# kubernetes-sigs/karpenter

Hardware: AMD Instinct MI355X
Metric: pods scheduled/sec (Solve()) (higher is better)
Workload: dtype int64

## Files before the change

### karpenter_amd/csrc/fast_engine.h

```cpp
#pragma once
#include <type_traits>
#include "kernels.h"
#include "pdq_emul.h"

namespace ks {

constexpr int kFastRows = 4;
constexpr uint32_t kFastFree = 0xFFFFFFFFu;
constexpr uint32_t kFastLastBit = 0x80000000u;
constexpr int kFastEnt = 1024;
constexpr int kFastPool = 256;
constexpr int kFastMaxPareto = 16;
constexpr int kFastMaxVar = 12;
constexpr uint64_t kFastExtBit = 1ull << 63;
constexpr int kFastVarBits = 56;

struct FastClaim { uint64_t vmask; int32_t req[4]; };
template <int R> struct FastRec { uint64_t vmask; int32_t req[4]; uint64_t acc[R]; };
struct FastSlot { uint64_t cvmask; uint64_t dmask; int32_t size[4]; uint32_t tmplok; uint32_t kdef; };
struct FastEnt { uint64_t vmask; int32_t cap[4]; uint32_t info; uint32_t pad; };

struct FastPlan {
  int total_bytes, cap;
  int off_state, off_key, off_ord, off_snap, off_ent, off_pool, off_slot, off_misc, off_hot;
// ... 40 lines not shown
  uint16_t* o_snap;
  uint64_t* c_rec;
  uint32_t* cls_first;
  uint32_t* cls_last;
  uint32_t* max_active;
  FastNodes* nodes;
  uint32_t* nd_pod;
  const uint64_t* nd_dead0;
  FastPlan plan;
  int enabled;
};

typedef uint64_t __attribute__((may_alias)) u64_alias;
template <class T>
KS_FN T lds_get(const KS_LDS T* p) {
  static_assert(sizeof(T) % 8 == 0, "lds_get: 8-byte multiples");
  T out;
  u64_alias* o = (u64_alias*)&out;
  const KS_LDS u64_alias* s = (const KS_LDS u64_alias*)p;
#pragma unroll
  for (int i = 0; i < (int)(sizeof(T) / 8); ++i) o[i] = s[i];
  return out;
}
template <class T>
KS_FN void lds_put(KS_LDS T* p, const T& v) {
  static_assert(sizeof(T) % 8 == 0, "lds_put: 8-byte multiples");
  const u64_alias* o = (const u64_alias*)&v;
  KS_LDS u64_alias* s = (KS_LDS u64_alias*)p;
#pragma unroll
  for (int i = 0; i < (int)(sizeof(T) / 8); ++i) s[i] = o[i];
}


typedef uint32_t __attribute__((vector_size(16), may_alias)) u32x4_alias;
template <class T>
KS_FN T lds_get16(const KS_LDS T* p) {
  static_assert(sizeof(T) % 16 == 0, "lds_get16: 16-byte multiples");
  T out;
  u32x4_alias* o = (u32x4_alias*)&out;
  const KS_LDS u32x4_alias* s = (const KS_LDS u32x4_alias*)p;
#pragma unroll
  for (int i = 0; i < (int)(sizeof(T) / 16); ++i) o[i] = s[i];
  return out;
}
KS_FN FastEnt ent_live(const KS_LDS FastEnt* p) {
  FastEnt out;
  *(u32x4_alias*)&out = *(const KS_LDS u32x4_alias*)p;
  *(u64_alias*)&out.cap[2] = *(const KS_LDS u64_alias*)&p->cap[2];
  out.info = 1; out.pad = 0;
  return out;
}
template <class T>
KS_FN void lds_put16(KS_LDS T* p, const T& v) {
  static_assert(sizeof(T) % 16 == 0, "lds_put16: 16-byte multiples");
  const u32x4_alias* o = (const u32x4_alias*)&v;
  KS_LDS u32x4_alias* s = (KS_LDS u32x4_alias*)p;
#pragma unroll
  for (int i = 0; i < (int)(sizeof(T) / 16); ++i) s[i] = o[i];
}

template <bool HBM, int R> struct ClaimRecs;
template <int R> struct ClaimRecs<false, R> {
  KS_LDS FastRec<R>* p;
  KS_FN FastClaim state(uint32_t c) const { return lds_get((const KS_LDS FastClaim*)&p[c]); }
  KS_FN void put_state(uint32_t c, const FastClaim& v) const { lds_put((KS_LDS FastClaim*)&p[c], v); }
  KS_FN uint64_t acc(uint32_t c, int row) const { return p[c].acc[row]; }
  KS_FN void put_acc(uint32_t c, int row, uint64_t v) const { p[c].acc[row] = v; }
// ... 167 lines not shown
  uint32_t helper;
  uint32_t simd[4];
};
#if KS_DEVICE
KS_FN uint32_t mail_load(const KS_LDS uint32_t* p) { return *(const volatile KS_LDS uint32_t*)p; }
KS_FN void mail_store(KS_LDS uint32_t* p, uint32_t v) { *(volatile KS_LDS uint32_t*)p = v; }
#else
KS_FN uint32_t mail_load(const uint32_t* p) { return *p; }
KS_FN void mail_store(uint32_t* p, uint32_t v) { *p = v; }
#endif

struct FastHot {
  alignas(16) FastMail mail;
  int base, bi, bn, n, np, max_steps, steps, status;
  int pend_a, pend_x, pend_new, ev_arg;
  uint32_t pend_mv;
  int rf_x;
  int rf_x2;
  unsigned long long n_steps, n_tests, n_ref, hot_cycles;
  unsigned long long tsec[8];
  unsigned long long hw[4];
  const uint32_t* q_class; const volatile int* cancel; uint32_t* q_claim; uint32_t* q_cnt;
  uint32_t cur[kFastRows][64];
  uint32_t scls[kFastRows][64];
  uint32_t bcls[64], oclaim[64], ocnt[64], nxt_cls[64];
};

template <class W, int GS, int R>
struct FastCold {
  const ProblemView* Pk;
  const Workspace* Sk;
  const FastWork* Fk;
  typedef typename FastMem<GS, R>::o16 o16;
  ClaimOrder<W, o16, false> order;
  typename FastMem<GS, R>::s16 snap;
  typename FastMem<GS, R>::States cst;
  KS_LDS FastEnt* ent;
  KS_LDS int32_t* pool;
  KS_LDS FastSlot* aslot;
  KS_LDS FastMisc* Mp;
  KS_LDS FastHot* hs;
  int n_claims = 0, nv = 0, n_ent = 0, n_pool = 0, n_evict = 0;
  uint32_t host_seq = 0, active_templates = 0;
  int bail_code = 0;
  int lo_ = 0, hi_ = -1;
  unsigned long long n_ref_extra = 0, n_cold_tests = 0;

  KS_DEV void init(const ProblemView* p, const Workspace* s, const FastWork* f, char* lds) {
    Pk = p; Sk = s; Fk = f;
    const FastPlan& pl = f->plan;
    Mp = (KS_LDS FastMisc*)(lds + pl.off_misc);
    hs = (KS_LDS FastHot*)(lds + pl.off_hot);
    if constexpr (GS >= 1) cst.p = (FastRec<R>*)f->c_rec; else cst.p = (KS_LDS FastRec<R>*)(lds + pl.off_state);
    typedef typename FastMem<GS, R>::s16 s16;
    if constexpr (GS >= 2) { order.key = (o16)f->o_key; order.ord = (o16)f->o_ord; }
    else { order.key = (o16)(lds + pl.off_key); order.ord = (o16)(lds + pl.off_ord); }
    if constexpr (GS >= 1) snap = (s16)f->o_snap; else snap = (s16)(lds + pl.off_snap);
    order.pos = nullptr;
    ent = (KS_LDS FastEnt*)(lds + pl.off_ent);
    pool = (KS_LDS int32_t*)(lds + pl.off_pool);
    aslot = (KS_LDS FastSlot*)(lds + pl.off_slot);
  }

  KS_COLD int create_entry(uint64_t vm) {
    vm = W::uniform(vm);
    const ProblemView& P = *Pk; const Workspace& S = *Sk; const FastWork& F = *Fk;
    const int t = (int)(vm >> 56);
    const int iw = P.it_words, n_its = P.n_its, nr = P.n_res;
    const Dict& d = P.dict;
    const ProblemView& Pv = P;
    KS_LDS FastMisc& Mm = *Mp;
    const uint64_t* tits = S.t_its + (size_t)t * iw;
    KS_LDS uint64_t* its = Mp->its;
    const int nvv = nv;
    W::for_n(iw, [&](int w) {
      uint64_t acc = tits[w];
      for (int j = 0; j < nvv; ++j) {
        const int k = Mm.vkey[j];
        if (!((Pv.it_keys >> k) & 1u)) continue;
// ... 309 lines not shown
      while (todo) {
        LaneVar<uint64_t> missv;
        const uint64_t td = todo;
        uint64_t okb = 0, miss = 0, d0, d1;
        W::ballot4([&](int l) {
          missv.at(l) = 0;
          if (!((td >> l) & 1)) return 0;
          const FastClaim st = cs_.state((uint32_t)(x0 + l));
          if (!((rec.tmplok >> (st.vmask >> 56)) & 1u)) return 0;
          const uint64_t m = st.vmask & rec.cvmask;
          if (!fast_fields_ok(m, rec.dmask)) return 0;
          FastEnt e;
          if (fast_lookup(ent, m, e) < 0) { missv.at(l) = m; return 2; }
          return fast_fits(pool, e, st.req, rec.size) ? 1 : 0;
        }, okb, miss, d0, d1);
        accm |= okb;
        todo = miss;
        if (miss && create_entry(missv.bcast(ctz64(miss))) < 0) { bail_code = DECLINE_CACHE_FULL; return -1; }
      }
      W::each([&](int l) {
        if (x0 + l < nc) {
          const uint64_t w = cs_.acc((uint32_t)(x0 + l), row);
          cs_.put_acc((uint32_t)(x0 + l), row, (w & ~bit) | (((accm >> l) & 1) ? bit : 0ull));
        }
      });
    }
    W::sync();
    return slot | evicted;
  }

  KS_COLD void slow_sort(int n, int defect, int app) {
    order.n = (int)W::uniform((uint64_t)(uint32_t)n); order.defect = (int)W::uniform((uint64_t)(uint32_t)defect); order.defect_append = W::uniform((uint64_t)app) != 0;
    n = order.n;
    const o16 oo = order.ord; const typename FastMem<GS, R>::s16 sn = snap;
    if constexpr (FastMem<GS, R>::kSnapHbm) {
      W::copy8(sn, oo, n);
      order.sort();
      lo_ = W::find_first8(0, n, [&](int i) { return sn[i] != oo[i]; });
      if (lo_ >= n) { lo_ = 0; hi_ = -1; return; }
      hi_ = W::find_last8(0, n, [&](int i) { return sn[i] != oo[i]; });
    } else {
      const int n8 = (n + 7) >> 3;
      const KS_LDS u32x4_alias* const o8 = (const KS_LDS u32x4_alias*)oo;
      KS_LDS u32x4_alias* const s8 = (KS_LDS u32x4_alias*)sn;
      W::for_n(n8, [&](int i) { s8[i] = o8[i]; });
      order.sort();
      auto differs = [&](int i) { const u32x4_alias a = s8[i], b = o8[i]; return ((a[0] ^ b[0]) | (a[1] ^ b[1]) | (a[2] ^ b[2]) | (a[3] ^ b[3])) != 0; };
      const int c0 = W::find_first(0, n8, differs);
      if (c0 >= n8) { lo_ = 0; hi_ = -1; return; }
      const int c1 = W::find_last(0, n8, differs);
      lo_ = W::find_first(c0 * 8, c0 * 8 + 8 < n ? c0 * 8 + 8 : n, [&](int i) { return sn[i] != oo[i]; });
      hi_ = W::find_last(c1 * 8, c1 * 8 + 8 < n ? c1 * 8 + 8 : n, [&](int i) { return sn[i] != oo[i]; });
    }
  }
  KS_DEV void shift_right16(KS_LDS uint16_t* arr, int b, int a) {
    KS_LDS u32x4_alias* const v = (KS_LDS u32x4_alias*)arr;
    const KS_LDS uint32_t* const dw = (const KS_LDS uint32_t*)arr;
    for (int e0 = a & ~511; e0 >= 0 && e0 + 511 >= b; e0 -= 512) {
      LaneVar<uint32_t> d0, d1, d2, d3, pv;
      const uint32_t below = e0 > 0 ? dw[(e0 >> 1) - 1] : 0u;
      W::each([&](int l) {
        const int e = e0 + 8 * l;
        d0.at(l) = 0; d1.at(l) = 0; d2.at(l) = 0; d3.at(l) = 0;
        if (e <= a && e + 7 >= b) { const u32x4_alias x = v[(e0 >> 3) + l]; d0.at(l) = x[0]; d1.at(l) = x[1]; d2.at(l) = x[2]; d3.at(l) = x[3]; }
      });
      LaneVar<uint32_t> up;
      W::each([&](int l) { up.at(l) = d3.shuffle(l, (l + 63) & 63); });
// ... 80 lines not shown
    }
    bail_code = DECLINE_UNSCHEDULABLE_POD;
    return 0;
  }

  KS_COLD void finish(int status, int n, unsigned long long steps, unsigned long long n_steps, unsigned long long n_tests, unsigned long long n_ref, const unsigned long long* tc) {
    const Workspace& S = *Sk; const FastWork& F = *Fk;
    if (status != 3 && status != 1) {
      uint32_t* go = S.o_ord;
      const o16 oo = order.ord; const o16 ok_ = order.key;
      FastClaim* gs = F.c_state; uint32_t* gn = F.c_npods; uint16_t* ge = F.c_ent;
      const typename FastMem<GS, R>::States ls = cst;
      const KS_LDS FastEnt* en = ent;
      W::for_n(n, [&](int i) { const uint32_t c = oo[i]; go[i] = c; gn[c] = ok_[i]; });
      W::for_n(n, [&](int c) {
        const FastClaim st = ls.state((uint32_t)c);
        FastEnt e;
        gs[c] = st;
        ge[c] = (uint16_t)fast_lookup(en, st.vmask, e);
      });
      W::store(S.n_claims_out, n_claims);
    }
    FastNodes nd{};
    if (F.nodes) nd = *F.nodes;
    if (status == 0 && nd.limit_hit) status = 2;
    if (status) W::store(S.status_out, status);
    Counters c{};
    c.bin_evaluations = n_tests + n_cold_tests + nd.n_tests; c.full_evaluations = n_steps; c.queue_pops = steps + nd.n_placed; c.sorts = steps; c.slow_sorts = order.slow_sorts;
    c.column_resets = (unsigned long long)n_evict; c.ref_bin_evaluations = n_ref + n_ref_extra + nd.n_ref;
    c.decline = (unsigned long long)(bail_code > 0 ? bail_code : 0);
    if (tc) for (int i = 0; i < 16; ++i) c.cycles[i] = tc[i];
#ifdef KSOLVE_PHASE_TIMERS
    for (int i = 0; i < 4; ++i) c.cycles[16 + i] = hs->hw[i];
    c.cycles[18] = (hs->hw[2] << 32) | (unsigned long long)(hs->mail.simd[0] | (hs->mail.simd[1] << 8) | (hs->mail.simd[2] << 16) | (hs->mail.simd[3] << 24));
#endif
    if (F.nodes) c.cycles[19] = (unsigned long long)nd.variant;
    if (W::leader()) *S.counters = c;
    W::sync();
  }
};

template <int GS, int R>
struct FastHotCtx {
  typename FastMem<GS, R>::o16 okey, oord; typename FastMem<GS, R>::States cst; KS_LDS FastEnt* ent; KS_LDS int32_t* pool;
  KS_LDS FastSlot* aslot; KS_LDS FastHot* hs;
};
enum { FEV_DONE = 0, FEV_REFRESH = 1, FEV_SLOT = 2, FEV_SLOWSORT = 3, FEV_PLACE = 4, FEV_NEWCLAIM = 5, FEV_COUNT = 6, FEV_SLOW = 7, FEV_CONT = 8, FEV_DEAD = 9 };

template <int R>
struct FastHelperK {
  LaneVar<uint32_t> tok[R];
  LaneVar<uint64_t> cvm[R], dm[R], gd[R];
  LaneVar<int32_t> z0[R], z1[R], z2[R], z3[R];
  uint32_t gen = 0xFFFFFFFFu, miss = 0;
};
template <class W, int R>
KS_FN void fast_helper_consts(FastHelperK<R>& k, const KS_LDS FastSlot* aslot, const KS_LDS FastHot* hs) {
  W::each([&](int l) {
#pragma unroll
    for (int j = 0; j < R; ++j) {
      const FastSlot s = lds_get(&aslot[j * 64 + l]);
      k.cvm[j].at(l) = s.cvmask; k.dm[j].at(l) = s.dmask; k.gd[j].at(l) = (s.dmask << 1) & ~s.dmask;
      k.z0[j].at(l) = s.size[0]; k.z1[j].at(l) = s.size[1]; k.z2[j].at(l) = s.size[2]; k.z3[j].at(l) = s.size[3];
      k.tok[j].at(l) = hs->scls[j][l] == kFastFree ? 0u : s.tmplok;
    }
  });
// ... 991 lines not shown
```

### karpenter_amd/csrc/pdq_emul.h

```cpp
#pragma once
#include "wave.h"

namespace ks {

template <class W, class P32 = KS_LDS uint32_t*, bool POS = true>
struct ClaimOrder {
  P32 key;
  P32 ord;
  P32 pos;
  int n = 0;
  int defect = -1;
  bool defect_append = false;
  uint64_t slow_sorts = 0;

  KS_FN uint32_t position(int c) const { return pos[c]; }
  KS_FN uint32_t claim_at(int i) const { return ord[i]; }
  KS_FN bool less(int i, int j) const { return key[i] < key[j]; }
  KS_FN void swap(int i, int j) {
    if (i == j) return;
    uint32_t ki = key[i], kj = key[j], oi = ord[i], oj = ord[j];
    W::store(&key[i], kj); W::store(&key[j], ki);
    W::store(&ord[i], oj); W::store(&ord[j], oi);
    if constexpr (POS) { W::store(&pos[oj], (uint32_t)i); W::store(&pos[oi], (uint32_t)j); }
    W::sync();
  }
  KS_FN void rotate_right(int to, int from) {
    if (to >= from) return;
    uint32_t mk = key[from], mo = ord[from];
    for (int top = from; top > to; top -= kRound) {
      int lo = top - kRound > to ? top - kRound : to;
      shift_round(lo, top, +1, false);
    }
    W::store(&key[to], mk); W::store(&ord[to], mo); if constexpr (POS) W::store(&pos[mo], (uint32_t)to);
    W::sync();
  }
  KS_FN void rotate_left(int from, int to, bool same_keys = false) {
    if (to <= from) return;
    uint32_t mk = key[from], mo = ord[from];
// ... 13 lines not shown
  KS_FN void shift_round(int lo, int hi, int delta, bool same_keys) {
#if KS_DEVICE
    uint32_t k[kPerLane], o[kPerLane];
    if (same_keys) {
#pragma unroll
      for (int j = 0; j < kPerLane; ++j) { const int i = lo + j * 64 + W::lane(); if (i < hi) o[j] = ord[i]; }
      W::sync();
#pragma unroll
      for (int j = 0; j < kPerLane; ++j) { const int i = lo + j * 64 + W::lane(); if (i < hi) { ord[i + delta] = o[j]; if constexpr (POS) pos[o[j]] = (uint32_t)(i + delta); } }
      W::sync();
      return;
    }
#pragma unroll
    for (int j = 0; j < kPerLane; ++j) { const int i = lo + j * 64 + W::lane(); if (i < hi) { k[j] = key[i]; o[j] = ord[i]; } }
    W::sync();
#pragma unroll
    for (int j = 0; j < kPerLane; ++j) { const int i = lo + j * 64 + W::lane(); if (i < hi) { key[i + delta] = k[j]; ord[i + delta] = o[j]; if constexpr (POS) pos[o[j]] = (uint32_t)(i + delta); } }
    W::sync();
#else
    if (delta > 0) for (int i = hi - 1; i >= lo; --i) { if (!same_keys) key[i + 1] = key[i]; ord[i + 1] = ord[i]; if constexpr (POS) pos[ord[i + 1]] = i + 1; }
    else for (int i = lo; i < hi; ++i) { if (!same_keys) key[i - 1] = key[i]; ord[i - 1] = ord[i]; if constexpr (POS) pos[ord[i - 1]] = i - 1; }
#endif
  }
  KS_FN int lower_bound_sorted(int lo, int hi, uint32_t v) const {
    while (lo < hi) { const int mid = lo + (hi - lo) / 2; if (key[mid] < v) lo = mid + 1; else hi = mid; }
    return lo;
  }
  KS_FN int upper_last_sorted(int lo, int hi, uint32_t v) const {
    int a = lo, b = hi;
    while (a < b) { const int mid = a + (b - a) / 2; if (!(v < key[mid])) a = mid + 1; else b = mid; }
    return a - 1;
  }

  KS_FN void increment(int claim) {
    int p = (int)pos[claim];
    W::store(&key[p], key[p] + 1);
    W::sync();
    defect = p; defect_append = false;
  }
  KS_FN void append(int claim) {
    W::store(&key[n], 1u); W::store(&ord[n], (uint32_t)claim); if constexpr (POS) W::store(&pos[claim], (uint32_t)n);
    W::sync();
    defect = n; defect_append = true;
    n++;
  }

  static KS_FN int bits_len(unsigned x) { return x ? 32 - __builtin_clz(x) : 0; }

  KS_FN void insertion_sort(int a, int b) {
    for (int i = a + 1; i < b; i++)
      for (int j = i; j > a && less(j, j - 1); j--) swap(j, j - 1);
  }
  KS_FN void sift_down(int lo, int hi, int first) {
    int root = lo;
    for (;;) {
      int child = 2 * root + 1;
      if (child >= hi) return;
      if (child + 1 < hi && less(first + child, first + child + 1)) child++;
      if (!less(first + root, first + child)) return;
      swap(first + root, first + child);
      root = child;
    }
  }
  KS_FN void heap_sort(int a, int b) {
    int first = a, lo = 0, hi = b - a;
    for (int i = (hi - 1) / 2; i >= 0; i--) sift_down(i, hi, first);
    for (int i = hi - 1; i >= 0; i--) { swap(first, first + i); sift_down(lo, i, first); }
  }
  static KS_FN void order2(int& a, int& b, uint32_t& ka, uint32_t& kb, int& swaps) {
    if (kb < ka) { swaps++; int t = a; a = b; b = t; uint32_t tk = ka; ka = kb; kb = tk; }
  }
  static KS_FN void median3(int a, int b, int c, uint32_t ka, uint32_t kb, uint32_t kc, int& swaps, int& out, uint32_t& kout) {
    order2(a, b, ka, kb, swaps); order2(b, c, kb, kc, swaps); order2(a, b, ka, kb, swaps);
    out = b; kout = kb;
  }
  KS_FN int choose_pivot(int a, int b, int& hint) {
    int l = b - a, swaps = 0;
    int i = a + l / 4 * 1, j = a + l / 4 * 2, k = a + l / 4 * 3;
    if (l >= 8) {
      uint32_t ki, kj, kk;
      if (l >= 50) {
        uint32_t s0 = key[i - 1], s1 = key[i], s2 = key[i + 1], s3 = key[j - 1], s4 = key[j], s5 = key[j + 1], s6 = key[k - 1], s7 = key[k], s8 = key[k + 1];
        int oi, oj, ok;
        median3(i - 1, i, i + 1, s0, s1, s2, swaps, oi, ki);
        median3(j - 1, j, j + 1, s3, s4, s5, swaps, oj, kj);
        median3(k - 1, k, k + 1, s6, s7, s8, swaps, ok, kk);
        i = oi; j = oj; k = ok;
      } else { ki = key[i]; kj = key[j]; kk = key[k]; }
      int oj2; uint32_t dummy;
      median3(i, j, k, ki, kj, kk, swaps, oj2, dummy);
      j = oj2;
    }
    hint = swaps == 0 ? 1 : (swaps == 12 ? 2 : 0);
    return j;
  }
  KS_FN void reverse_range(int a, int b) { int i = a, j = b - 1; while (i < j) { swap(i, j); i++; j--; } }

  KS_FN int next_descent(int i, int b, bool top) {
    if (top) {
      if (defect < 0) return b;
      for (int x = defect; x <= defect + 1; ++x) if (x >= i && x >= 1 && x < b && key[x] < key[x - 1]) return x;
      return b;
    }
    const P32 kp = key;
    return ff(i, b, [kp](int x) { return kp[x] < kp[x - 1]; });
  }
  KS_FN bool partial_insertion_sort(int a, int b, bool top) {
    int i = a + 1;
    for (int step = 0; step < 5; step++) {
      i = next_descent(i, b, top);
      if (i == b) return true;
      if (b - a < 50) return false;
      if (top) {
        const P32 kq = key;
        if (defect_append) {
          uint32_t mv = key[i];
          int t = fl(0, i, [kq, mv](int x) { return !(mv < kq[x]); });
          rotate_right(t + 1, i);
        } else {
          uint32_t mv = key[i - 1];
          int e = ff(i, b, [kq, mv](int x) { return !(kq[x] < mv); });
          rotate_left(i - 1, e - 1);
        }
        defect = -1;
        return true;
      }
      swap(i, i - 1);
      if (i - a >= 2) {
        uint32_t mv = key[i - 1];
        const P32 kp = key;
        int t = fl(0, i - 1, [kp, mv](int x) { return !(mv < kp[x]); });
        rotate_right(t + 1, i - 1);
      }
      if (b - i >= 2) {
        uint32_t mv = key[i];
        const P32 kp = key;
        int e = ff(i + 1, b, [kp, mv](int x) { return !(kp[x] < mv); });
        rotate_left(i, e - 1);
      }
      if (top) defect = -1;
    }
    return false;
  }
  KS_FN void break_patterns(int a, int b) {
    int length = b - a;
    if (length >= 8) {
      uint64_t r = (uint64_t)length;
      unsigned modulus = 1u << bits_len((unsigned)length);
      int idx = a + (length / 4) * 2 - 1;
      for (int t = 0; t < 3; t++) {
        r ^= r << 13; r ^= r >> 7; r ^= r << 17;
        int other = (int)((unsigned)r & (modulus - 1));
        if (other >= length) other -= length;
        swap(idx - 1 + t, a + other);
      }
    }
  }
  KS_FN int partition_equal(int a, int b, int pivot) {
    swap(a, pivot);
    uint32_t pv = key[a];
    const P32 kp = key;
    int i = a + 1, j = b - 1;
    for (;;) {
      i = ff(i, j + 1, [kp, pv](int x) { return pv < kp[x]; });
      j = fl(i, j + 1, [kp, pv](int x) { return !(pv < kp[x]); });
      if (i > j) break;
      swap(i, j); i++; j--;
    }
    return i;
  }
  KS_FN int partition(int a, int b, int pivot, bool& already) {
    swap(a, pivot);
    uint32_t pv = key[a];
    const P32 kp = key;
    int i = a + 1, j = b - 1;
    i = ff(i, j + 1, [kp, pv](int x) { return !(kp[x] < pv); });
    j = fl(i, j + 1, [kp, pv](int x) { return kp[x] < pv; });
    if (i > j) { swap(j, a); already = true; return j; }
    swap(i, j); i++; j--;
    for (;;) {
      i = ff(i, j + 1, [kp, pv](int x) { return !(kp[x] < pv); });
      j = fl(i, j + 1, [kp, pv](int x) { return kp[x] < pv; });
      if (i > j) break;
      swap(i, j); i++; j--;
    }
    swap(j, a);
    already = false;
    return j;
  }

  struct Frame { int a, b, limit; bool was_balanced, was_partitioned; };

  KS_FN void pdqsort(int a0, int b0, int limit0) {
    Frame stack[40];
    int sp = 0;
    Frame cur{a0, b0, limit0, true, true};
    bool top = true;
    for (;;) {
      bool done = false;
      for (;;) {
        int a = cur.a, b = cur.b;
        int length = b - a;
        if (length <= 12) { insertion_sort(a, b); done = true; break; }
        if (cur.limit == 0) { heap_sort(a, b); done = true; break; }
        if (!cur.was_balanced) { break_patterns(a, b); cur.limit--; }
        int hint;
        int pivot = choose_pivot(a, b, hint);
        if (hint == 2) { reverse_range(a, b); pivot = (b - 1) - (pivot - a); hint = 1; top = false; }
        if (cur.was_balanced && cur.was_partitioned && hint == 1) {
          if (partial_insertion_sort(a, b, top)) { done = true; break; }
        }
        if (top) slow_sorts++;
        top = false;
        if (a > 0 && !less(a - 1, pivot)) { cur.a = partition_equal(a, b, pivot); continue; }
        bool already;
        int mid = partition(a, b, pivot, already);
        cur.was_partitioned = already;
        int left_len = mid - a, right_len = b - mid;
        int balance_threshold = length / 8;
        Frame child;
        if (left_len < right_len) {
          cur.was_balanced = left_len >= balance_threshold;
          child = Frame{a, mid, cur.limit, true, true};
          cur.a = mid + 1;
        } else {
          cur.was_balanced = right_len >= balance_threshold;
          child = Frame{mid + 1, b, cur.limit, true, true};
          cur.b = mid;
        }
        stack[sp++] = cur;
        cur = child;
      }
      (void)done;
      if (sp == 0) break;
      cur = stack[--sp];
    }
  }

  KS_FN void sort() {
    if (defect < 0 || n <= 1) { defect = -1; return; }
    if (n <= 12) {
      if (defect_append) {
        uint32_t mv = key[n - 1];
        const P32 kp = key;
        int t = fl(0, n - 1, [kp, mv](int x) { return !(mv < kp[x]); });
        rotate_right(t + 1, n - 1);
      } else {
        int p = defect;
        uint32_t mv = key[p];
        const P32 kp = key;
        int e = ff(p + 1, n, [kp, mv](int x) { return !(kp[x] < mv); });
        rotate_left(p, e - 1, true);
      }
      defect = -1;
      return;
    }
    if (n >= 50) {
      const int q = n / 4, p = defect;
      const bool sampled = (p >= q - 1 && p <= q + 1) || (p >= 2 * q - 1 && p <= 2 * q + 1) || (p >= 3 * q - 1 && p <= 3 * q + 1);
      if (!sampled) {
        const P32 kq = key;
        if (defect_append) {
          const int i = n - 1;
          if (i >= 1 && key[i] < key[i - 1]) {
            const uint32_t mv = key[i];
            const int t = kPerLane > 1 ? upper_last_sorted(0, i, mv) : fl(0, i, [kq, mv](int x) { return !(mv < kq[x]); });
            rotate_right(t + 1, i);
          }
        } else if (p + 1 < n && key[p + 1] < key[p]) {
          const uint32_t mv = key[p];
          const int e = kPerLane > 1 ? lower_bound_sorted(p + 1, n, mv) : ff(p + 1, n, [kq, mv](int x) { return !(kq[x] < mv); });
          rotate_left(p, e - 1, true);
        }
        defect = -1;
        return;
      }
    }
    pdqsort(0, n, bits_len((unsigned)n));
    defect = -1;
  }
};

}
```

### karpenter_amd/csrc/wave.h

```cpp
#pragma once
#include <stdint.h>

#if defined(__HIPCC__) && !defined(KSOLVE_HOST_EMULATION)
#define KS_DEVICE 1
#define KS_FN __host__ __device__ __forceinline__
#define KS_DEV __device__ __forceinline__
#define KS_LDS __attribute__((address_space(3)))
#define KS_GLOBAL __attribute__((address_space(1)))
#else
#define KS_DEVICE 0
#define KS_FN inline
#define KS_DEV inline
#define KS_LDS
#define KS_GLOBAL
#endif

namespace ks {

#if KS_DEVICE

struct Wave {
  KS_DEV static int lane() { return (int)(threadIdx.x & 63); }
  KS_DEV static uint64_t uniform(uint64_t v) {
    const uint32_t lo = (uint32_t)__builtin_amdgcn_readfirstlane((int)(uint32_t)v), hi = (uint32_t)__builtin_amdgcn_readfirstlane((int)(uint32_t)(v >> 32));
// ... 277 lines not shown
    static_assert(sizeof(T) == 4 || sizeof(T) == 8, "LaneVar::shuffle: 32- or 64-bit values");
    if constexpr (sizeof(T) == 4) {
      const int x = __builtin_amdgcn_ds_bpermute(src << 2, __builtin_bit_cast(int, v));
      return __builtin_bit_cast(T, x);
    } else {
      const uint64_t u = __builtin_bit_cast(uint64_t, v);
      const uint32_t lo = (uint32_t)__builtin_amdgcn_ds_bpermute(src << 2, (int)(uint32_t)u);
      const uint32_t hi = (uint32_t)__builtin_amdgcn_ds_bpermute(src << 2, (int)(uint32_t)(u >> 32));
      return __builtin_bit_cast(T, (uint64_t)lo | ((uint64_t)hi << 32));
    }
  }
  KS_DEV T bcast(int lane) const {
    static_assert(sizeof(T) == 4 || sizeof(T) == 8, "LaneVar: 32- or 64-bit values");
    if constexpr (sizeof(T) == 4) {
      const int x = __builtin_amdgcn_readlane(__builtin_bit_cast(int, v), lane);
      return __builtin_bit_cast(T, x);
    } else {
      const uint64_t u = __builtin_bit_cast(uint64_t, v);
      const uint32_t lo = (uint32_t)__builtin_amdgcn_readlane((int)(uint32_t)u, lane);
      const uint32_t hi = (uint32_t)__builtin_amdgcn_readlane((int)(uint32_t)(u >> 32), lane);
      return __builtin_bit_cast(T, (uint64_t)lo | ((uint64_t)hi << 32));
    }
  }
#else
  T v[64];
  T& at(int l) { return v[l]; }
  T v_of(int l) const { return v[l]; }
  void set(int lane, T x) { v[lane] = x; }
  T shuffle(int, int src) const { return v[src & 63]; }
  T bcast(int lane) const { return v[lane]; }
#endif
};

KS_FN int popc64(uint64_t x) { return __builtin_popcountll(x); }
KS_FN int ctz64(uint64_t x) { return __builtin_ctzll(x); }

}
```

Baseline: 1.545 million.

## Sort small claim orders in wave registers and add wide 16-bit LDS scans

Pulls the pdqsort logic out into a generic PdqSort template. A new register-resident RegOrder backend sorts orders of at most 64 claims in lane registers using ballots and shuffles, instead of touching LDS for every compare and swap. It also adds a wide scan path that reads packed 16-bit keys from LDS 8 per lane for the non-HBM ClaimOrder. The goal is to cut LDS traffic and per-element loop latency in slow_sort. The cost is more broadcast and readlane work on each swap, and more register pressure.

```diff
diff --git a/karpenter_amd/csrc/fast_engine.h b/karpenter_amd/csrc/fast_engine.h
--- a/karpenter_amd/csrc/fast_engine.h
+++ b/karpenter_amd/csrc/fast_engine.h
@@ -96,7 +96,6 @@
 }
 
 
-typedef uint32_t __attribute__((vector_size(16), may_alias)) u32x4_alias;
 template <class T>
 KS_FN T lds_get16(const KS_LDS T* p) {
   static_assert(sizeof(T) % 16 == 0, "lds_get16: 16-byte multiples");
@@ -330,7 +329,7 @@
   const Workspace* Sk;
   const FastWork* Fk;
   typedef typename FastMem<GS, R>::o16 o16;
-  ClaimOrder<W, o16, false> order;
+  ClaimOrder<W, o16, false, !FastMem<GS, R>::kOrderHbm> order;
   typename FastMem<GS, R>::s16 snap;
   typename FastMem<GS, R>::States cst;
   KS_LDS FastEnt* ent;
@@ -343,6 +342,9 @@
   int bail_code = 0;
   int lo_ = 0, hi_ = -1;
   unsigned long long n_ref_extra = 0, n_cold_tests = 0;
+#ifdef KSOLVE_PHASE_TIMERS
+  unsigned long long t_small = 0, n_small = 0;
+#endif
 
   KS_DEV void init(const ProblemView* p, const Workspace* s, const FastWork* f, char* lds) {
     Pk = p; Sk = s; Fk = f;
@@ -718,7 +720,25 @@
   KS_COLD void slow_sort(int n, int defect, int app) {
     order.n = (int)W::uniform((uint64_t)(uint32_t)n); order.defect = (int)W::uniform((uint64_t)(uint32_t)defect); order.defect_append = W::uniform((uint64_t)app) != 0;
     n = order.n;
+#ifdef KSOLVE_PHASE_TIMERS
+    const unsigned long long t_in = W::clock();
+#endif
     const o16 oo = order.ord; const typename FastMem<GS, R>::s16 sn = snap;
+    if (n <= 64) {
+      RegOrder<W> r;
+      r.load(order.key, oo, n);
+      r.defect = order.defect; r.defect_append = order.defect_append;
+      const LaneVar<uint32_t> before = r.o;
+      r.sort();
+      order.slow_sorts += r.slow_sorts; order.defect = -1;
+      const uint64_t moved = W::ballot([&](int l) { return l < n && before.v_of(l) != r.o.v_of(l); });
+      r.store(order.key, oo);
+      lo_ = moved ? ctz64(moved) : 0; hi_ = moved ? 63 - __builtin_clzll(moved) : -1;
+#ifdef KSOLVE_PHASE_TIMERS
+      t_small += W::clock() - t_in; n_small++;
+#endif
+      return;
+    }
     if constexpr (FastMem<GS, R>::kSnapHbm) {
       W::copy8(sn, oo, n);
       order.sort();
@@ -865,6 +885,7 @@
     if (tc) for (int i = 0; i < 16; ++i) c.cycles[i] = tc[i];
 #ifdef KSOLVE_PHASE_TIMERS
     for (int i = 0; i < 4; ++i) c.cycles[16 + i] = hs->hw[i];
+    c.cycles[20] = t_small | (n_small << 44);
     c.cycles[18] = (hs->hw[2] << 32) | (unsigned long long)(hs->mail.simd[0] | (hs->mail.simd[1] << 8) | (hs->mail.simd[2] << 16) | (hs->mail.simd[3] << 24));
 #endif
     if (F.nodes) c.cycles[19] = (unsigned long long)nd.variant;
diff --git a/karpenter_amd/csrc/pdq_emul.h b/karpenter_amd/csrc/pdq_emul.h
--- a/karpenter_amd/csrc/pdq_emul.h
+++ b/karpenter_amd/csrc/pdq_emul.h
@@ -3,7 +3,244 @@
 
 namespace ks {
 
-template <class W, class P32 = KS_LDS uint32_t*, bool POS = true>
+struct PdqFrame { int a, b, limit; bool was_balanced, was_partitioned; };
+struct PdqFrameArray {
+  PdqFrame f[40];
+  KS_FN void push(int sp, const PdqFrame& x) { f[sp] = x; }
+  KS_FN PdqFrame pop(int sp) const { return f[sp]; }
+};
+
+template <class S>
+struct PdqSort {
+  static KS_FN int bits_len(unsigned x) { return x ? 32 - __builtin_clz(x) : 0; }
+
+  static KS_FN void insertion_sort(S& s, int a, int b) {
+    for (int i = a + 1; i < b; i++)
+      for (int j = i; j > a && s.less(j, j - 1); j--) s.swap(j, j - 1);
+  }
+  static KS_FN void sift_down(S& s, int lo, int hi, int first) {
+    int root = lo;
+    for (;;) {
+      int child = 2 * root + 1;
+      if (child >= hi) return;
+      if (child + 1 < hi && s.less(first + child, first + child + 1)) child++;
+      if (!s.less(first + root, first + child)) return;
+      s.swap(first + root, first + child);
+      root = child;
+    }
+  }
+  static KS_FN void heap_sort(S& s, int a, int b) {
+    int first = a, lo = 0, hi = b - a;
+    for (int i = (hi - 1) / 2; i >= 0; i--) sift_down(s, i, hi, first);
+    for (int i = hi - 1; i >= 0; i--) { s.swap(first, first + i); sift_down(s, lo, i, first); }
+  }
+  static KS_FN void order2(int& a, int& b, uint32_t& ka, uint32_t& kb, int& swaps) {
+    if (kb < ka) { swaps++; int t = a; a = b; b = t; uint32_t tk = ka; ka = kb; kb = tk; }
+  }
+  static KS_FN void median3(int a, int b, int c, uint32_t ka, uint32_t kb, uint32_t kc, int& swaps, int& out, uint32_t& kout) {
+    order2(a, b, ka, kb, swaps); order2(b, c, kb, kc, swaps); order2(a, b, ka, kb, swaps);
+    out = b; kout = kb;
+  }
+  static KS_FN int choose_pivot(S& s, int a, int b, int& hint) {
+    int l = b - a, swaps = 0;
+    int i = a + l / 4 * 1, j = a + l / 4 * 2, k = a + l / 4 * 3;
+    if (l >= 8) {
+      uint32_t ki, kj, kk;
+      if (l >= 50) {
+        uint32_t s0 = s.key_at(i - 1), s1 = s.key_at(i), s2 = s.key_at(i + 1), s3 = s.key_at(j - 1), s4 = s.key_at(j), s5 = s.key_at(j + 1), s6 = s.key_at(k - 1), s7 = s.key_at(k), s8 = s.key_at(k + 1);
+        int oi, oj, ok;
+        median3(i - 1, i, i + 1, s0, s1, s2, swaps, oi, ki);
+        median3(j - 1, j, j + 1, s3, s4, s5, swaps, oj, kj);
+        median3(k - 1, k, k + 1, s6, s7, s8, swaps, ok, kk);
+        i = oi; j = oj; k = ok;
+      } else { ki = s.key_at(i); kj = s.key_at(j); kk = s.key_at(k); }
+      int oj2; uint32_t dummy;
+      median3(i, j, k, ki, kj, kk, swaps, oj2, dummy);
+      j = oj2;
+    }
+    hint = swaps == 0 ? 1 : (swaps == 12 ? 2 : 0);
+    return j;
+  }
+  static KS_FN void reverse_range(S& s, int a, int b) { int i = a, j = b - 1; while (i < j) { s.swap(i, j); i++; j--; } }
+
+  static KS_FN int next_descent(S& s, int i, int b, bool top) {
+    if (top) {
+      if (s.defect < 0) return b;
+      for (int x = s.defect; x <= s.defect + 1; ++x) if (x >= i && x >= 1 && x < b && s.key_at(x) < s.key_at(x - 1)) return x;
+      return b;
+    }
+    return s.first_descent(i, b);
+  }
+  static KS_FN bool partial_insertion_sort(S& s, int a, int b, bool top) {
+    int i = a + 1;
+    for (int step = 0; step < 5; step++) {
+      i = next_descent(s, i, b, top);
+      if (i == b) return true;
+      if (b - a < 50) return false;
+      if (top) {
+        if (s.defect_append) {
+          uint32_t mv = s.key_at(i);
+          int t = s.last_le(0, i, mv);
+          s.rotate_right(t + 1, i);
+        } else {
+          uint32_t mv = s.key_at(i - 1);
+          int e = s.first_ge(i, b, mv);
+          s.rotate_left(i - 1, e - 1);
+        }
+        s.defect = -1;
+        return true;
+      }
+      s.swap(i, i - 1);
+      if (i - a >= 2) {
+        uint32_t mv = s.key_at(i - 1);
+        int t = s.last_le(0, i - 1, mv);
+        s.rotate_right(t + 1, i - 1);
+      }
+      if (b - i >= 2) {
+        uint32_t mv = s.key_at(i);
+        int e = s.first_ge(i + 1, b, mv);
+        s.rotate_left(i, e - 1);
+      }
+      if (top) s.defect = -1;
+    }
+    return false;
+  }
+  static KS_FN void break_patterns(S& s, int a, int b) {
+    int length = b - a;
+    if (length >= 8) {
+      uint64_t r = (uint64_t)length;
+      unsigned modulus = 1u << bits_len((unsigned)length);
+      int idx = a + (length / 4) * 2 - 1;
+      for (int t = 0; t < 3; t++) {
+        r ^= r << 13; r ^= r >> 7; r ^= r << 17;
+        int other = (int)((unsigned)r & (modulus - 1));
+        if (other >= length) other -= length;
+        s.swap(idx - 1 + t, a + other);
+      }
+    }
+  }
+  static KS_FN int partition_equal(S& s, int a, int b, int pivot) {
+    s.swap(a, pivot);
+    uint32_t pv = s.key_at(a);
+    int i = a + 1, j = b - 1;
+    for (;;) {
+      i = s.first_gt(i, j + 1, pv);
+      j = s.last_le(i, j + 1, pv);
+      if (i > j) break;
+      s.swap(i, j); i++; j--;
+    }
+    return i;
+  }
+  static KS_FN int partition(S& s, int a, int b, int pivot, bool& already) {
+    s.swap(a, pivot);
+    uint32_t pv = s.key_at(a);
+    int i = a + 1, j = b - 1;
+    i = s.first_ge(i, j + 1, pv);
+    j = s.last_lt(i, j + 1, pv);
+    if (i > j) { s.swap(j, a); already = true; return j; }
+    s.swap(i, j); i++; j--;
+    for (;;) {
+      i = s.first_ge(i, j + 1, pv);
+      j = s.last_lt(i, j + 1, pv);
+      if (i > j) break;
+      s.swap(i, j); i++; j--;
+    }
+    s.swap(j, a);
+    already = false;
+    return j;
+  }
+
+  typedef PdqFrame Frame;
+
+  static KS_FN void pdqsort(S& s, int a0, int b0, int limit0) {
+    typename S::FrameStack stack;
+    int sp = 0;
+    Frame cur{a0, b0, limit0, true, true};
+    bool top = true;
+    for (;;) {
+      bool done = false;
+      for (;;) {
+        int a = cur.a, b = cur.b;
+        int length = b - a;
+        if (length <= 12) { insertion_sort(s, a, b); done = true; break; }
+        if (cur.limit == 0) { heap_sort(s, a, b); done = true; break; }
+        if (!cur.was_balanced) { break_patterns(s, a, b); cur.limit--; }
+        int hint;
+        int pivot = choose_pivot(s, a, b, hint);
+        if (hint == 2) { reverse_range(s, a, b); pivot = (b - 1) - (pivot - a); hint = 1; top = false; }
+        if (cur.was_balanced && cur.was_partitioned && hint == 1) {
+          if (partial_insertion_sort(s, a, b, top)) { done = true; break; }
+        }
+        if (top) s.slow_sorts++;
+        top = false;
+        if (a > 0 && !s.less(a - 1, pivot)) { cur.a = partition_equal(s, a, b, pivot); continue; }
+        bool already;
+        int mid = partition(s, a, b, pivot, already);
+        cur.was_partitioned = already;
+        int left_len = mid - a, right_len = b - mid;
+        int balance_threshold = length / 8;
+        Frame child;
+        if (left_len < right_len) {
+          cur.was_balanced = left_len >= balance_threshold;
+          child = Frame{a, mid, cur.limit, true, true};
+          cur.a = mid + 1;
+        } else {
+          cur.was_balanced = right_len >= balance_threshold;
+          child = Frame{mid + 1, b, cur.limit, true, true};
+          cur.b = mid;
+        }
+        stack.push(sp++, cur);
+        cur = child;
+      }
+      (void)done;
+      if (sp == 0) break;
+      cur = stack.pop(--sp);
+    }
+  }
+
+  static KS_FN void sort(S& s) {
+    const int n = s.n;
+    if (s.defect < 0 || n <= 1) { s.defect = -1; return; }
+    if (n <= 12) {
+      if (s.defect_append) {
+        uint32_t mv = s.key_at(n - 1);
+        int t = s.last_le(0, n - 1, mv);
+        s.rotate_right(t + 1, n - 1);
+      } else {
+        int p = s.defect;
+        uint32_t mv = s.key_at(p);
+        int e = s.first_ge(p + 1, n, mv);
+        s.rotate_left(p, e - 1, true);
+      }
+      s.defect = -1;
+      return;
+    }
+    if (n >= 50) {
+      const int q = n / 4, p = s.defect;
+      const bool sampled = (p >= q - 1 && p <= q + 1) || (p >= 2 * q - 1 && p <= 2 * q + 1) || (p >= 3 * q - 1 && p <= 3 * q + 1);
+      if (!sampled) {
+        if (s.defect_append) {
+          const int i = n - 1;
+          if (i >= 1 && s.key_at(i) < s.key_at(i - 1)) {
+            const uint32_t mv = s.key_at(i);
+            const int t = s.last_le_sorted(0, i, mv);
+            s.rotate_right(t + 1, i);
+          }
+        } else if (p + 1 < n && s.key_at(p + 1) < s.key_at(p)) {
+          const uint32_t mv = s.key_at(p);
+          const int e = s.first_ge_sorted(p + 1, n, mv);
+          s.rotate_left(p, e - 1, true);
+        }
+        s.defect = -1;
+        return;
+      }
+    }
+    pdqsort(s, 0, n, bits_len((unsigned)n));
+    s.defect = -1;
+  }
+};
+
+template <class W, class P32 = KS_LDS uint32_t*, bool POS = true, bool WIDE = false>
 struct ClaimOrder {
   P32 key;
   P32 ord;
@@ -83,6 +320,63 @@
     return a - 1;
   }
 
+  KS_FN uint32_t key_at(int i) const { return key[i]; }
+  typedef PdqFrameArray FrameStack;
+  template <bool LAST, bool PREV, class F> KS_FN int scan(int lo, int hi, F pred) const {
+    if constexpr (WIDE) return wide_scan<LAST, PREV>(lo, hi, pred);
+    else {
+      const P32 kp = key;
+      auto at = [kp, pred](int x) { return pred((uint32_t)kp[x], PREV ? (uint32_t)kp[x - 1] : 0u); };
+      if constexpr (LAST) return fl(lo, hi, at); else return ff(lo, hi, at);
+    }
+  }
+  KS_FN int first_ge(int lo, int hi, uint32_t v) const { return scan<false, false>(lo, hi, [v](uint32_t k, uint32_t) { return !(k < v); }); }
+  KS_FN int first_gt(int lo, int hi, uint32_t v) const { return scan<false, false>(lo, hi, [v](uint32_t k, uint32_t) { return v < k; }); }
+  KS_FN int last_le(int lo, int hi, uint32_t v) const { return scan<true, false>(lo, hi, [v](uint32_t k, uint32_t) { return !(v < k); }); }
+  KS_FN int last_lt(int lo, int hi, uint32_t v) const { return scan<true, false>(lo, hi, [v](uint32_t k, uint32_t) { return k < v; }); }
+  KS_FN int first_descent(int lo, int hi) const { return scan<false, true>(lo, hi, [](uint32_t k, uint32_t below) { return k < below; }); }
+  template <bool LAST, bool PREV, class F> KS_FN int wide_scan(int lo, int hi, F pred) const {
+    if (lo >= hi) return LAST ? lo - 1 : hi;
+    const int rlo = PREV ? lo - 1 : lo;
+    const auto pieces = pieces16(key);
+    const P32 kp = key;
+    const int base_lo = rlo & ~511, base_hi = (hi - 1) & ~511;
+    for (int base = LAST ? base_hi : base_lo; LAST ? base >= base_lo : base <= base_hi; base += LAST ? -512 : 512) {
+      LaneVar<uint32_t> w0, w1, w2, w3, dn, m8;
+      const uint32_t under = (PREV && base > 0) ? (uint32_t)kp[base - 1] : 0u;
+      W::each([&](int l) {
+        const int e = base + 8 * l;
+        w0.at(l) = 0; w1.at(l) = 0; w2.at(l) = 0; w3.at(l) = 0;
+        if (e < hi && e + 7 >= rlo) { const u32x4_alias x = pieces[(base >> 3) + l]; w0.at(l) = x[0]; w1.at(l) = x[1]; w2.at(l) = x[2]; w3.at(l) = x[3]; }
+      });
+      if constexpr (PREV) {
+        LaneVar<uint32_t> up;
+        W::each([&](int l) { up.at(l) = w3.shuffle(l, (l + 63) & 63); });
+        W::each([&](int l) { dn.at(l) = l ? up.at(l) >> 16 : under; });
+      }
+      W::each([&](int l) {
+        const int e = base + 8 * l;
+        const uint32_t w[4] = {w0.at(l), w1.at(l), w2.at(l), w3.at(l)};
+        uint32_t below = 0, m = 0;
+        if constexpr (PREV) below = dn.at(l);
+#pragma unroll
+        for (int j = 0; j < 8; ++j) { const uint32_t kx = (w[j >> 1] >> (16 * (j & 1))) & 0xFFFFu; m |= (pred(kx, below) ? 1u : 0u) << j; below = kx; }
+        const int a = lo - e, b = hi - e;
+        const uint32_t in = (b >= 8 ? 0xFFu : b <= 0 ? 0u : (1u << b) - 1u) & (a <= 0 ? 0xFFu : a >= 8 ? 0u : (0xFFu << a) & 0xFFu);
+        m8.at(l) = m & in;
+      });
+      const uint64_t any = W::ballot([&](int l) { return m8.at(l) != 0; });
+      if (any) {
+        const int who = LAST ? 63 - __builtin_clzll(any) : ctz64(any);
+        const uint32_t bits = m8.bcast(who);
+        return base + 8 * who + (LAST ? 31 - __builtin_clz(bits) : __builtin_ctz(bits));
+      }
+    }
+    return LAST ? lo - 1 : hi;
+  }
+  KS_FN int first_ge_sorted(int lo, int hi, uint32_t v) const { return kPerLane > 1 ? lower_bound_sorted(lo, hi, v) : first_ge(lo, hi, v); }
+  KS_FN int last_le_sorted(int lo, int hi, uint32_t v) const { return kPerLane > 1 ? upper_last_sorted(lo, hi, v) : last_le(lo, hi, v); }
+
   KS_FN void increment(int claim) {
     int p = (int)pos[claim];
     W::store(&key[p], key[p] + 1);
@@ -96,240 +390,75 @@
     n++;
   }
 
-  static KS_FN int bits_len(unsigned x) { return x ? 32 - __builtin_clz(x) : 0; }
-
-  KS_FN void insertion_sort(int a, int b) {
-    for (int i = a + 1; i < b; i++)
-      for (int j = i; j > a && less(j, j - 1); j--) swap(j, j - 1);
-  }
-  KS_FN void sift_down(int lo, int hi, int first) {
-    int root = lo;
-    for (;;) {
-      int child = 2 * root + 1;
-      if (child >= hi) return;
-      if (child + 1 < hi && less(first + child, first + child + 1)) child++;
-      if (!less(first + root, first + child)) return;
-      swap(first + root, first + child);
-      root = child;
-    }
-  }
-  KS_FN void heap_sort(int a, int b) {
-    int first = a, lo = 0, hi = b - a;
-    for (int i = (hi - 1) / 2; i >= 0; i--) sift_down(i, hi, first);
-    for (int i = hi - 1; i >= 0; i--) { swap(first, first + i); sift_down(lo, i, first); }
-  }
-  static KS_FN void order2(int& a, int& b, uint32_t& ka, uint32_t& kb, int& swaps) {
-    if (kb < ka) { swaps++; int t = a; a = b; b = t; uint32_t tk = ka; ka = kb; kb = tk; }
-  }
-  static KS_FN void median3(int a, int b, int c, uint32_t ka, uint32_t kb, uint32_t kc, int& swaps, int& out, uint32_t& kout) {
-    order2(a, b, ka, kb, swaps); order2(b, c, kb, kc, swaps); order2(a, b, ka, kb, swaps);
-    out = b; kout = kb;
-  }
-  KS_FN int choose_pivot(int a, int b, int& hint) {
-    int l = b - a, swaps = 0;
-    int i = a + l / 4 * 1, j = a + l / 4 * 2, k = a + l / 4 * 3;
-    if (l >= 8) {
-      uint32_t ki, kj, kk;
-      if (l >= 50) {
-        uint32_t s0 = key[i - 1], s1 = key[i], s2 = key[i + 1], s3 = key[j - 1], s4 = key[j], s5 = key[j + 1], s6 = key[k - 1], s7 = key[k], s8 = key[k + 1];
-        int oi, oj, ok;
-        median3(i - 1, i, i + 1, s0, s1, s2, swaps, oi, ki);
-        median3(j - 1, j, j + 1, s3, s4, s5, swaps, oj, kj);
-        median3(k - 1, k, k + 1, s6, s7, s8, swaps, ok, kk);
-        i = oi; j = oj; k = ok;
-      } else { ki = key[i]; kj = key[j]; kk = key[k]; }
-      int oj2; uint32_t dummy;
-      median3(i, j, k, ki, kj, kk, swaps, oj2, dummy);
-      j = oj2;
-    }
-    hint = swaps == 0 ? 1 : (swaps == 12 ? 2 : 0);
-    return j;
-  }
-  KS_FN void reverse_range(int a, int b) { int i = a, j = b - 1; while (i < j) { swap(i, j); i++; j--; } }
-
-  KS_FN int next_descent(int i, int b, bool top) {
-    if (top) {
-      if (defect < 0) return b;
-      for (int x = defect; x <= defect + 1; ++x) if (x >= i && x >= 1 && x < b && key[x] < key[x - 1]) return x;
-      return b;
-    }
-    const P32 kp = key;
-    return ff(i, b, [kp](int x) { return kp[x] < kp[x - 1]; });
-  }
-  KS_FN bool partial_insertion_sort(int a, int b, bool top) {
-    int i = a + 1;
-    for (int step = 0; step < 5; step++) {
-      i = next_descent(i, b, top);
-      if (i == b) return true;
-      if (b - a < 50) return false;
-      if (top) {
-        const P32 kq = key;
-        if (defect_append) {
-          uint32_t mv = key[i];
-          int t = fl(0, i, [kq, mv](int x) { return !(mv < kq[x]); });
-          rotate_right(t + 1, i);
-        } else {
-          uint32_t mv = key[i - 1];
-          int e = ff(i, b, [kq, mv](int x) { return !(kq[x] < mv); });
-          rotate_left(i - 1, e - 1);
-        }
-        defect = -1;
-        return true;
-      }
-      swap(i, i - 1);
-      if (i - a >= 2) {
-        uint32_t mv = key[i - 1];
-        const P32 kp = key;
-        int t = fl(0, i - 1, [kp, mv](int x) { return !(mv < kp[x]); });
-        rotate_right(t + 1, i - 1);
-      }
-      if (b - i >= 2) {
-        uint32_t mv = key[i];
-        const P32 kp = key;
-        int e = ff(i + 1, b, [kp, mv](int x) { return !(kp[x] < mv); });
-        rotate_left(i, e - 1);
-      }
-      if (top) defect = -1;
-    }
-    return false;
-  }
-  KS_FN void break_patterns(int a, int b) {
-    int length = b - a;
-    if (length >= 8) {
-      uint64_t r = (uint64_t)length;
-      unsigned modulus = 1u << bits_len((unsigned)length);
-      int idx = a + (length / 4) * 2 - 1;
-      for (int t = 0; t < 3; t++) {
-        r ^= r << 13; r ^= r >> 7; r ^= r << 17;
-        int other = (int)((unsigned)r & (modulus - 1));
-        if (other >= length) other -= length;
-        swap(idx - 1 + t, a + other);
-      }
-    }
-  }
-  KS_FN int partition_equal(int a, int b, int pivot) {
-    swap(a, pivot);
-    uint32_t pv = key[a];
-    const P32 kp = key;
-    int i = a + 1, j = b - 1;
-    for (;;) {
-      i = ff(i, j + 1, [kp, pv](int x) { return pv < kp[x]; });
-      j = fl(i, j + 1, [kp, pv](int x) { return !(pv < kp[x]); });
-      if (i > j) break;
-      swap(i, j); i++; j--;
-    }
-    return i;
-  }
-  KS_FN int partition(int a, int b, int pivot, bool& already) {
-    swap(a, pivot);
-    uint32_t pv = key[a];
-    const P32 kp = key;
-    int i = a + 1, j = b - 1;
-    i = ff(i, j + 1, [kp, pv](int x) { return !(kp[x] < pv); });
-    j = fl(i, j + 1, [kp, pv](int x) { return kp[x] < pv; });
-    if (i > j) { swap(j, a); already = true; return j; }
-    swap(i, j); i++; j--;
-    for (;;) {
-      i = ff(i, j + 1, [kp, pv](int x) { return !(kp[x] < pv); });
-      j = fl(i, j + 1, [kp, pv](int x) { return kp[x] < pv; });
-      if (i > j) break;
-      swap(i, j); i++; j--;
-    }
-    swap(j, a);
-    already = false;
-    return j;
-  }
-
-  struct Frame { int a, b, limit; bool was_balanced, was_partitioned; };
-
-  KS_FN void pdqsort(int a0, int b0, int limit0) {
-    Frame stack[40];
-    int sp = 0;
-    Frame cur{a0, b0, limit0, true, true};
-    bool top = true;
-    for (;;) {
-      bool done = false;
-      for (;;) {
-        int a = cur.a, b = cur.b;
-        int length = b - a;
-        if (length <= 12) { insertion_sort(a, b); done = true; break; }
-        if (cur.limit == 0) { heap_sort(a, b); done = true; break; }
-        if (!cur.was_balanced) { break_patterns(a, b); cur.limit--; }
-        int hint;
-        int pivot = choose_pivot(a, b, hint);
-        if (hint == 2) { reverse_range(a, b); pivot = (b - 1) - (pivot - a); hint = 1; top = false; }
-        if (cur.was_balanced && cur.was_partitioned && hint == 1) {
-          if (partial_insertion_sort(a, b, top)) { done = true; break; }
-        }
-        if (top) slow_sorts++;
-        top = false;
-        if (a > 0 && !less(a - 1, pivot)) { cur.a = partition_equal(a, b, pivot); continue; }
-        bool already;
-        int mid = partition(a, b, pivot, already);
-        cur.was_partitioned = already;
-        int left_len = mid - a, right_len = b - mid;
-        int balance_threshold = length / 8;
-        Frame child;
-        if (left_len < right_len) {
-          cur.was_balanced = left_len >= balance_threshold;
-          child = Frame{a, mid, cur.limit, true, true};
-          cur.a = mid + 1;
-        } else {
-          cur.was_balanced = right_len >= balance_threshold;
-          child = Frame{mid + 1, b, cur.limit, true, true};
-          cur.b = mid;
-        }
-        stack[sp++] = cur;
-        cur = child;
-      }
-      (void)done;
-      if (sp == 0) break;
-      cur = stack[--sp];
-    }
-  }
-
-  KS_FN void sort() {
-    if (defect < 0 || n <= 1) { defect = -1; return; }
-    if (n <= 12) {
-      if (defect_append) {
-        uint32_t mv = key[n - 1];
-        const P32 kp = key;
-        int t = fl(0, n - 1, [kp, mv](int x) { return !(mv < kp[x]); });
-        rotate_right(t + 1, n - 1);
-      } else {
-        int p = defect;
-        uint32_t mv = key[p];
-        const P32 kp = key;
-        int e = ff(p + 1, n, [kp, mv](int x) { return !(kp[x] < mv); });
-        rotate_left(p, e - 1, true);
-      }
-      defect = -1;
-      return;
-    }
-    if (n >= 50) {
-      const int q = n / 4, p = defect;
-      const bool sampled = (p >= q - 1 && p <= q + 1) || (p >= 2 * q - 1 && p <= 2 * q + 1) || (p >= 3 * q - 1 && p <= 3 * q + 1);
-      if (!sampled) {
-        const P32 kq = key;
-        if (defect_append) {
-          const int i = n - 1;
-          if (i >= 1 && key[i] < key[i - 1]) {
-            const uint32_t mv = key[i];
-            const int t = kPerLane > 1 ? upper_last_sorted(0, i, mv) : fl(0, i, [kq, mv](int x) { return !(mv < kq[x]); });
-            rotate_right(t + 1, i);
-          }
-        } else if (p + 1 < n && key[p + 1] < key[p]) {
-          const uint32_t mv = key[p];
-          const int e = kPerLane > 1 ? lower_bound_sorted(p + 1, n, mv) : ff(p + 1, n, [kq, mv](int x) { return !(kq[x] < mv); });
-          rotate_left(p, e - 1, true);
-        }
-        defect = -1;
-        return;
-      }
-    }
-    pdqsort(0, n, bits_len((unsigned)n));
-    defect = -1;
-  }
+  KS_FN void sort() { PdqSort<ClaimOrder>::sort(*this); }
 };
 
+template <class W>
+struct RegOrder {
+  LaneVar<uint32_t> k, o;
+  int n = 0;
+  int defect = -1;
+  bool defect_append = false;
+  uint64_t slow_sorts = 0;
+
+  template <class P> KS_FN void load(P key, P ord, int n_) {
+    n = n_;
+    W::each([&](int l) { const int i = l < n_ ? l : 0; k.at(l) = key[i]; o.at(l) = ord[i]; });
+  }
+  template <class P> KS_FN void store(P key, P ord) {
+    const int n_ = n;
+    W::each([&](int l) { if (l < n_) { key[l] = k.at(l); ord[l] = o.at(l); } });
+    W::sync();
+  }
+  KS_FN uint32_t key_at(int i) const { return k.bcast(i); }
+  struct FrameStack {
+    LaneVar<uint32_t> v;
+    KS_FN void push(int sp, const PdqFrame& x) { v.set(sp, (uint32_t)x.a | ((uint32_t)x.b << 7) | ((uint32_t)x.limit << 14) | ((uint32_t)x.was_balanced << 18) | ((uint32_t)x.was_partitioned << 19)); }
+    KS_FN PdqFrame pop(int sp) const {
+      const uint32_t p = v.bcast(sp);
+      return PdqFrame{(int)(p & 127u), (int)((p >> 7) & 127u), (int)((p >> 14) & 15u), ((p >> 18) & 1u) != 0, ((p >> 19) & 1u) != 0};
+    }
+  };
+  KS_FN bool less(int i, int j) const { return k.bcast(i) < k.bcast(j); }
+  KS_FN void swap(int i, int j) {
+    if (i == j) return;
+    const uint32_t ki = k.bcast(i), kj = k.bcast(j), oi = o.bcast(i), oj = o.bcast(j);
+    W::each([&](int l) { k.at(l) = l == i ? kj : l == j ? ki : k.at(l); o.at(l) = l == i ? oj : l == j ? oi : o.at(l); });
+  }
+  template <class F> KS_FN void permute(F src) {
+    LaneVar<uint32_t> tk, to;
+    W::each([&](int l) { const int from = src(l); tk.at(l) = k.shuffle(l, from); to.at(l) = o.shuffle(l, from); });
+    W::each([&](int l) { k.at(l) = tk.at(l); o.at(l) = to.at(l); });
+  }
+  KS_FN void rotate_right(int to, int from) {
+    if (to >= from) return;
+    permute([to, from](int l) { return l == to ? from : (l > to && l <= from) ? l - 1 : l; });
+  }
+  KS_FN void rotate_left(int from, int to, bool = false) {
+    if (to <= from) return;
+    permute([to, from](int l) { return l == to ? from : (l >= from && l < to) ? l + 1 : l; });
+  }
+  template <class F> KS_FN int first(int lo, int hi, F pred) const {
+    const uint64_t m = W::ballot([&](int l) { return l >= lo && l < hi && pred(l); });
+    return m ? ctz64(m) : hi;
+  }
+  template <class F> KS_FN int last(int lo, int hi, F pred) const {
+    const uint64_t m = W::ballot([&](int l) { return l >= lo && l < hi && pred(l); });
+    return m ? 63 - __builtin_clzll(m) : lo - 1;
+  }
+  KS_FN int first_ge(int lo, int hi, uint32_t v) const { return first(lo, hi, [&](int l) { return !(k.v_of(l) < v); }); }
+  KS_FN int first_gt(int lo, int hi, uint32_t v) const { return first(lo, hi, [&](int l) { return v < k.v_of(l); }); }
+  KS_FN int last_le(int lo, int hi, uint32_t v) const { return last(lo, hi, [&](int l) { return !(v < k.v_of(l)); }); }
+  KS_FN int last_lt(int lo, int hi, uint32_t v) const { return last(lo, hi, [&](int l) { return k.v_of(l) < v; }); }
+  KS_FN int first_descent(int lo, int hi) const {
+    LaneVar<uint32_t> below;
+    W::each([&](int l) { below.at(l) = k.shuffle(l, (l + 63) & 63); });
+    return first(lo, hi, [&](int l) { return l >= 1 && k.v_of(l) < below.v_of(l); });
+  }
+  KS_FN int first_ge_sorted(int lo, int hi, uint32_t v) const { return first_ge(lo, hi, v); }
+  KS_FN int last_le_sorted(int lo, int hi, uint32_t v) const { return last_le(lo, hi, v); }
+
+  KS_FN void sort() { PdqSort<RegOrder>::sort(*this); }
+};
+
 }
diff --git a/karpenter_amd/csrc/wave.h b/karpenter_amd/csrc/wave.h
--- a/karpenter_amd/csrc/wave.h
+++ b/karpenter_amd/csrc/wave.h
@@ -333,6 +333,9 @@
 #endif
 };
 
+typedef uint32_t __attribute__((vector_size(16), may_alias)) u32x4_alias;
+KS_FN const KS_LDS u32x4_alias* pieces16(const KS_LDS uint16_t* p) { return (const KS_LDS u32x4_alias*)p; }
+
 KS_FN int popc64(uint64_t x) { return __builtin_popcountll(x); }
 KS_FN int ctz64(uint64_t x) { return __builtin_ctzll(x); }
 
```

Measured after the change: 1.596 million (median of 6 runs). 1.03x the previous value.
